# kubewharf/kubebrain

Measured on NVIDIA H100. Metric: range-scan + watch-fanout events/sec, higher is better.
Workload: dtype u8

## Files before the change

### kubebrain_b200/csrc/kb_watch.cu

```cuda
#include <algorithm>
#include <map>
#include <unordered_map>

#include "kb_internal.cuh"

struct kb_events_dev {
    DBuf keys;
    DBuf klen;
    DBuf rev;
    DBuf batch_off;
    uint32_t n = 0, nb = 0, stride = 0;
};

struct WatchTablesDev {
    uint32_t n_ids = 0, n_groups = 0, n_lens = 0, table_size = 0, max_len = 0, pstride16 = 1;
    uint64_t d_hint = 0;
    DBuf gprefix, wgroup, wminrev, lens, table;
    DBuf gstate , galloc, lists, ematch, seg, seg_sorted, bitmaps, pm, wstate ,
        wstart, total;
    DBuf arena;
    size_t tab_end = 0, scr_bytes = 0, scr_sig = 0;
    bool scratch_clean = false;
    uint32_t scratch_groups = 0, scratch_large = 0, scratch_bm_words = 0;
    uint32_t fan_gen = 0;
    uint32_t fan_set = 0;
    int fan_grid = 0;
    uint32_t wr_set = 0;
    cudaEvent_t ev_fan = nullptr, ev_write[2] = {nullptr, nullptr};
};

namespace {

constexpr unsigned FULL = 0xffffffffu;
constexpr uint64_t FNV_OFFSET = 14695981039346656037ull;
constexpr uint64_t FNV_PRIME = 1099511628211ull;

__host__ __device__ __forceinline__ uint32_t slot_of(uint64_t h, uint32_t len, uint32_t mask)
{
    uint64_t m = h ^ ((uint64_t)len * 0x9E3779B97F4A7C15ull);
    m ^= m >> 29;
    return (uint32_t)(m ^ (m >> 32)) & mask;
}

struct EvDev {
    const uint4 *keys;
    const uint32_t *klen;
    const uint64_t *rev;
    const uint64_t *batch_off;
    uint32_t n, nb, stride16;
};

struct TabDev {
    const uint4 *gprefix;
    const uint32_t *wgroup;
    const uint64_t *wminrev;
    const uint32_t *lens;
    const uint4 *table;
    uint32_t n_ids, n_groups, n_lens, mask, max_len, pstride16;
};

enum { FC_NONMONO = 0, FC_CURSOR = 1, FC_NLARGE = 2, FC_NMED = 3, FC_ARRIVE = 4, FC_GEN = 5, FC_DONE = 6, FC_ABORT = 7, FC_WORDS = 16 };
constexpr unsigned long long FAN_UNSET = ~0ull, FAN_BUSY = ~0ull - 1;
constexpr uint32_t FAN_THREADS = 384;
constexpr uint32_t BM_WORDS = 256;

struct FanScratch {
    uint32_t *gcnt, *gfill, *ctl;
    unsigned long long *galloc;
    uint32_t *med_list, *large_list;
    uint32_t *ematch, *seg, *sorted, *bitmaps;
    uint64_t *pm;
    uint32_t *wcnt, *wsrc, *wn, *wlo;
    uint64_t *wstart, *total;
    uint32_t big_t, max_large, bm_words, chunks_per_group, gen_base;
    uint32_t *z_gcnt, *z_bitmaps, *nlarge_w, *nlarge_r;
    unsigned long long *z_galloc;
    uint64_t *o_start, *h_start;
    uint64_t *h_pub, epoch;
};

__device__ __forceinline__ uint32_t ldcg32(const uint32_t *p) { return __ldcg(p); }
__device__ __forceinline__ uint64_t ldcg64(const uint64_t *p) { return __ldcg((const unsigned long long *)p); }

__device__ __forceinline__ void fan_grid_sync(uint32_t *ctl, uint32_t target)
{
    __syncthreads();
    if (threadIdx.x == 0) {
        __threadfence();
        if (atomicAdd(&ctl[FC_ARRIVE], 1u) == gridDim.x - 1) {
            atomicExch(&ctl[FC_ARRIVE], 0u);
            __threadfence();
            atomicExch(&ctl[FC_GEN], target);
        } else {
            const long long t0 = clock64();
            while (*(volatile uint32_t *)&ctl[FC_GEN] != target) {
                __nanosleep(64);
                if (clock64() - t0 > 4000000000ll) {
                    atomicExch(&ctl[FC_ABORT], 1u);
                    break;
                }
                if (*(volatile uint32_t *)&ctl[FC_ABORT]) break;
            }
        }
        __threadfence();
    }
    __syncthreads();
}

__device__ __forceinline__ void d_batch_pm(const EvDev &ev, uint64_t *__restrict__ pm, uint32_t *__restrict__ nonmono,
                                           uint32_t vblock)
{
    const uint32_t w = (vblock * blockDim.x + threadIdx.x) >> 5, lane = threadIdx.x & 31;
    if (w >= ev.nb) return;
    const uint64_t lo = ev.batch_off[w], hi = ev.batch_off[w + 1];
    uint64_t carry = 0;
    bool bad = false;
    for (uint64_t c = lo; c < hi; c += 32) {
        const uint64_t i = c + lane;
        uint64_t v = i < hi ? ev.rev[i] : 0;
        if (i < hi && i > 0 && ev.rev[i - 1] > v) bad = true;
#pragma unroll
        for (int d = 1; d < 32; d <<= 1) {
            uint64_t o = __shfl_up_sync(FULL, v, d);
            if (lane >= (unsigned)d) v = max(v, o);
        }
        v = max(v, carry);
        if (i < hi) pm[i] = v;
        carry = __shfl_sync(FULL, v, 31);
    }
    if (__any_sync(FULL, bad) && lane == 0) atomicOr(nonmono, 1u);
}

constexpr int FAN_EPT = 3;

__device__ __forceinline__ void d_match_count(const EvDev &ev, const TabDev &tb, uint32_t *__restrict__ ematch,
                                              uint32_t *__restrict__ gcnt, uint32_t vblock)
{
    const uint32_t lane = threadIdx.x & 31;
    uint32_t i[FAN_EPT], klen[FAN_EPT];
    const uint4 *kp[FAN_EPT];
    uint64_t h[FAN_EPT];
    uint4 chunk[FAN_EPT];
    bool valid[FAN_EPT];
#pragma unroll
    for (int e = 0; e < FAN_EPT; e++) {
        i[e] = (vblock * FAN_EPT + e) * blockDim.x + threadIdx.x;
        valid[e] = i[e] < ev.n;
        klen[e] = valid[e] ? ev.klen[i[e]] : 0;
        kp[e] = ev.keys + (uint64_t)(valid[e] ? i[e] : 0) * ev.stride16;
        h[e] = FNV_OFFSET;
        chunk[e] = make_uint4(0, 0, 0, 0);
    }
    uint32_t pos = 0;
    for (uint32_t li = 0; li < tb.n_lens; li++) {
        const uint32_t L = __ldg(tb.lens + li);
        for (; pos < L; pos++) {
            if ((pos & 15) == 0) {
#pragma unroll
                for (int e = 0; e < FAN_EPT; e++) chunk[e] = __ldg(kp[e] + (pos >> 4));
            }
#pragma unroll
            for (int e = 0; e < FAN_EPT; e++) h[e] = (h[e] ^ (uint64_t)byte_of(chunk[e], pos & 15)) * FNV_PRIME;
        }
        uint32_t s[FAN_EPT], g[FAN_EPT];
        uint4 t[FAN_EPT];
#pragma unroll
        for (int e = 0; e < FAN_EPT; e++) {
            s[e] = slot_of(h[e], L, tb.mask);
            t[e] = __ldg(tb.table + s[e]);
            g[e] = KB_NONE;
        }
#pragma unroll
        for (int e = 0; e < FAN_EPT; e++) {
            if (!(valid[e] && L <= klen[e])) continue;
            for (;;) {
                if (t[e].w == KB_NONE) break;
                if (t[e].x == (uint32_t)h[e] && t[e].y == (uint32_t)(h[e] >> 32) && t[e].z == L) {
                    const uint4 *gp = tb.gprefix + (uint64_t)t[e].w * tb.pstride16;
                    bool eq = true;
                    for (uint32_t k = 0; k * 16 < L && eq; k++) {
                        uint4 a = __ldg(kp[e] + k), b = __ldg(gp + k);
                        int p = first_diff16(a, b);
                        if (p < 16 && k * 16 + p < L) eq = false;
                    }
                    if (eq) {
                        g[e] = t[e].w;
                        break;
                    }
                }
                s[e] = (s[e] + 1) & tb.mask;
                t[e] = __ldg(tb.table + s[e]);
            }
        }
#pragma unroll
        for (int e = 0; e < FAN_EPT; e++) {
            if (valid[e]) ematch[(uint64_t)li * ev.n + i[e]] = g[e];
            const unsigned peers = __match_any_sync(FULL, g[e]);
            if (g[e] != KB_NONE && lane == (unsigned)(__ffs(peers) - 1)) atomicAdd(&gcnt[g[e]], (uint32_t)__popc(peers));
        }
    }
}

__device__ __forceinline__ unsigned long long d_group_alloc(const FanScratch &sc, uint32_t g)
{
    unsigned long long a = __ldcg(&sc.galloc[g]);
    if (a < FAN_BUSY) return a;
    const unsigned long long old = atomicCAS(&sc.galloc[g], FAN_UNSET, FAN_BUSY);
    if (old == FAN_UNSET) {
        const uint32_t n = ldcg32(&sc.gcnt[g]);
        uint32_t cls = KB_NONE;
        if (n > sc.big_t) {
            const uint32_t slot = atomicAdd(&sc.ctl[FC_NLARGE], 1u);
            if (slot < sc.max_large) {
                cls = slot;
                sc.large_list[slot] = g;
            }
        } else if (n > 32) {
            sc.med_list[atomicAdd(&sc.ctl[FC_NMED], 1u)] = g;
        }
        const uint32_t base = atomicAdd(&sc.ctl[FC_CURSOR], n);
        a = ((unsigned long long)cls << 32) | base;
        __threadfence();
        atomicExch(&sc.galloc[g], a);
        return a;
    }
    if (old < FAN_BUSY) return old;
    do {
        __nanosleep(32);
        a = *(volatile unsigned long long *)&sc.galloc[g];
    } while (a >= FAN_BUSY);
    return a;
}

__device__ __forceinline__ void d_scatter(const FanScratch &sc, uint32_t n_events, uint32_t n_lens, uint32_t vblock)
{
    const uint32_t i = vblock * blockDim.x + threadIdx.x;
    const uint32_t lane = threadIdx.x & 31;
    const bool valid = i < n_events;
    for (uint32_t li = 0; li < n_lens; li++) {
        const uint32_t g = valid ? ldcg32(&sc.ematch[(uint64_t)li * n_events + i]) : KB_NONE;
        const unsigned peers = __match_any_sync(FULL, g);
        if (g == KB_NONE) continue;
        const uint32_t leader = __ffs(peers) - 1;
        unsigned long long a = 0;
        uint32_t fill = 0;
        if (lane == leader) {
            a = d_group_alloc(sc, g);
            if ((uint32_t)(a >> 32) == KB_NONE) fill = atomicAdd(&sc.gfill[g], (uint32_t)__popc(peers));
        }
        const uint32_t base = __shfl_sync(peers, (uint32_t)a, leader);
        const uint32_t cls = __shfl_sync(peers, (uint32_t)(a >> 32), leader);
        fill = __shfl_sync(peers, fill, leader);
        if (cls != KB_NONE) {
            if (lane == leader) sc.bitmaps[(uint64_t)cls * sc.bm_words + (i >> 5)] = peers;
        } else {
            sc.seg[base + fill + __popc(peers & ((1u << lane) - 1))] = i;
        }
    }
}

__device__ __forceinline__ uint32_t block_excl_scan_u32(uint32_t v, uint32_t *wsum , uint32_t &total)
{
    const uint32_t lane = threadIdx.x & 31, wid = threadIdx.x >> 5, nw = blockDim.x >> 5;
    uint32_t inc = v;
#pragma unroll
    for (int d = 1; d < 32; d <<= 1) {
        uint32_t o = __shfl_up_sync(FULL, inc, d);
        if (lane >= (unsigned)d) inc += o;
    }
    if (lane == 31) wsum[wid] = inc;
    __syncthreads();
    if (threadIdx.x == 0) {
        uint32_t run = 0;
        for (uint32_t k = 0; k < nw; k++) {
            uint32_t x = wsum[k];
            wsum[k] = run;
            run += x;
        }
        wsum[32] = run;
    }
    __syncthreads();
    const uint32_t ex = wsum[wid] + inc - v;
    total = wsum[32];
    __syncthreads();
    return ex;
}

__device__ __forceinline__ void d_sort_medium(const FanScratch &sc, uint32_t *bm, uint32_t *wsum, uint32_t *red)
{
    const uint32_t nmed = ldcg32(&sc.ctl[FC_NMED]);
    for (uint32_t bi = blockIdx.x; bi < nmed; bi += gridDim.x) {
        const uint32_t g = ldcg32(&sc.med_list[bi]);
        const uint32_t n = ldcg32(&sc.gcnt[g]), base = (uint32_t)__ldcg(&sc.galloc[g]);
        if (threadIdx.x == 0) {
            red[0] = 0xFFFFFFFFu;
            red[1] = 0;
        }
        __syncthreads();
        uint32_t mn = 0xFFFFFFFFu, mx = 0;
        for (uint32_t j = threadIdx.x; j < n; j += blockDim.x) {
            const uint32_t v = ldcg32(&sc.seg[base + j]);
            mn = min(mn, v);
            mx = max(mx, v);
        }
        atomicMin(&red[0], mn);
        atomicMax(&red[1], mx);
        __syncthreads();
        mn = red[0];
        mx = red[1];
        uint32_t outpos = 0;
        for (uint64_t w0 = mn & ~31u; w0 <= mx; w0 += (uint64_t)BM_WORDS * 32) {
            const uint64_t need_words = ((uint64_t)mx - w0) / 32 + 1;
            const uint32_t nwords = need_words < BM_WORDS ? (uint32_t)need_words : BM_WORDS;
            for (uint32_t j = threadIdx.x; j < nwords; j += blockDim.x) bm[j] = 0;
            __syncthreads();
            for (uint32_t j = threadIdx.x; j < n; j += blockDim.x) {
                const uint64_t v = ldcg32(&sc.seg[base + j]);
                if (v >= w0 && v < w0 + (uint64_t)nwords * 32) {
                    const uint32_t d = (uint32_t)(v - w0);
                    atomicOr(&bm[d >> 5], 1u << (d & 31));
                }
            }
            __syncthreads();
            const uint32_t per = (nwords + blockDim.x - 1) / blockDim.x;
            const uint32_t wlo = min(nwords, threadIdx.x * per), whi = min(nwords, wlo + per);
            uint32_t cnt = 0;
            for (uint32_t j = wlo; j < whi; j++) cnt += __popc(bm[j]);
            uint32_t total;
            uint32_t at = outpos + block_excl_scan_u32(cnt, wsum, total);
            for (uint32_t j = wlo; j < whi; j++) {
                uint32_t bits = bm[j];
                while (bits) {
                    const uint32_t b = __ffs(bits) - 1;
                    bits &= bits - 1;
                    sc.sorted[base + at++] = (uint32_t)(w0 + (uint64_t)j * 32 + b);
                }
            }
            outpos += total;
            __syncthreads();
        }
        __syncthreads();
    }
}

__device__ __forceinline__ void d_expand_large(const FanScratch &sc, uint32_t *wsum, uint32_t *pre_sp)
{
    uint32_t &pre_s = *pre_sp;
    const uint32_t nlarge = min(ldcg32(&sc.ctl[FC_NLARGE]), sc.max_large);
    for (uint32_t job = blockIdx.x; job < nlarge * sc.chunks_per_group; job += gridDim.x) {
        const uint32_t slot = job / sc.chunks_per_group, chunk = job % sc.chunks_per_group;
        const uint32_t g = ldcg32(&sc.large_list[slot]);
        const uint32_t *bm = sc.bitmaps + (uint64_t)slot * sc.bm_words;
        uint32_t part = 0;
        for (uint32_t j = threadIdx.x; j < chunk * FAN_THREADS; j += blockDim.x) part += __popc(ldcg32(&bm[j]));
        uint32_t tot;
        block_excl_scan_u32(part, wsum, tot);
        if (threadIdx.x == 0) pre_s = tot;
        __syncthreads();
        const uint32_t wi = chunk * FAN_THREADS + threadIdx.x;
        uint32_t bits = wi < sc.bm_words ? ldcg32(&bm[wi]) : 0;
        uint32_t total;
        uint32_t at = (uint32_t)__ldcg(&sc.galloc[g]) + pre_s + block_excl_scan_u32(__popc(bits), wsum, total);
        while (bits) {
            const uint32_t b = __ffs(bits) - 1;
            bits &= bits - 1;
            sc.sorted[at++] = wi * 32 + b;
        }
        __syncthreads();
    }
}

__device__ __forceinline__ void d_watcher_big(const TabDev &tb, const FanScratch &sc, bool mono, uint32_t w, uint32_t n,
                                              uint32_t base, uint32_t lane)
{
    const uint64_t mr = __ldg(tb.wminrev + w);
    uint32_t lo = 0, cnt = 0;
    if (n <= 32) {
        const uint32_t v = lane < n ? ldcg32(&sc.seg[base + lane]) : 0xFFFFFFFFu;
        uint32_t rank = 0;
#pragma unroll
        for (int j = 0; j < 32; j++) {
            const uint32_t o = __shfl_sync(FULL, v, j);
            rank += (o < v) ? 1u : 0u;
        }
        if (lane < n) sc.sorted[base + rank] = v;
        const bool keep = lane < n && ldcg64(&sc.pm[v]) >= mr;
        cnt = __popc(__ballot_sync(FULL, keep));
        lo = mono ? n - cnt : 0;
    } else if (mono) {
        const uint32_t *M = sc.sorted + base;
        uint32_t hi = n;
        for (;;) {
            const uint32_t span = hi - lo;
            if (span == 0) break;
            if (span <= 32) {
                const bool ge = lane < span && ldcg64(&sc.pm[ldcg32(&M[lo + lane])]) >= mr;
                const unsigned m = __ballot_sync(FULL, ge);
                lo += m ? (uint32_t)(__ffs(m) - 1) : span;
                break;
            }
            const uint32_t piv = lo + (uint32_t)(((uint64_t)span * (lane + 1)) / 33);
            const bool ge = ldcg64(&sc.pm[ldcg32(&M[piv])]) >= mr;
            const int k = __popc(~__ballot_sync(FULL, ge));
            uint32_t nlo = lo, nhi = hi;
            if (k > 0) nlo = __shfl_sync(FULL, piv, k - 1) + 1;
            if (k < 32) nhi = __shfl_sync(FULL, piv, k);
            lo = nlo;
            hi = nhi;
        }
        cnt = n - lo;
    } else {
        const uint32_t *M = sc.sorted + base;
        for (uint32_t c = 0; c < n; c += 32) {
            const uint32_t j = c + lane;
            const bool keep = j < n && ldcg64(&sc.pm[ldcg32(&M[j])]) >= mr;
            cnt += __popc(__ballot_sync(FULL, keep));
        }
    }
    if (lane == 0) {
        sc.wcnt[w] = cnt;
        sc.wsrc[w] = base;
        sc.wn[w] = n;
        sc.wlo[w] = lo;
    }
}

__device__ __forceinline__ void d_watcher_count(const TabDev &tb, const FanScratch &sc, bool mono)
{
    const uint32_t lane = threadIdx.x & 31, half = lane >> 4, sub = lane & 15;
    const uint32_t warps = (gridDim.x * blockDim.x) >> 5;
    for (uint32_t w0 = ((blockIdx.x * blockDim.x + threadIdx.x) >> 5) * 2; w0 < tb.n_ids; w0 += warps * 2) {
        const uint32_t w = w0 + half;
        const bool have = w < tb.n_ids;
        const uint32_t g = have ? __ldg(tb.wgroup + w) : KB_NONE;
        uint32_t n = 0, base = 0;
        unsigned long long a = FAN_UNSET;
        if (g != KB_NONE) a = __ldcg(&sc.galloc[g]);
        if (a < FAN_BUSY) {
            n = ldcg32(&sc.gcnt[g]);
            base = (uint32_t)a;
        }
        const unsigned hmask = half ? 0xFFFF0000u : 0x0000FFFFu;
        if (n <= 16) {
            const uint64_t mr = have ? __ldg(tb.wminrev + w) : 0;
            const uint32_t v = sub < n ? ldcg32(&sc.seg[base + sub]) : 0xFFFFFFFFu;
            uint32_t rank = 0;
#pragma unroll
            for (int j = 0; j < 16; j++) {
                const uint32_t o = __shfl_sync(hmask, v, j, 16);
                rank += (o < v) ? 1u : 0u;
            }
            if (sub < n) sc.sorted[base + rank] = v;
            const bool keep = sub < n && ldcg64(&sc.pm[v]) >= mr;
            const uint32_t cnt = __popc(__ballot_sync(hmask, keep));
            if (sub == 0 && have) {
                sc.wcnt[w] = cnt;
                sc.wsrc[w] = base;
                sc.wn[w] = n;
                sc.wlo[w] = mono ? n - cnt : 0;
            }
        }
        __syncwarp();
        const uint32_t n0 = __shfl_sync(FULL, n, 0), n1 = __shfl_sync(FULL, n, 16);
        const uint32_t b0 = __shfl_sync(FULL, base, 0), b1 = __shfl_sync(FULL, base, 16);
        if (n0 > 16) d_watcher_big(tb, sc, mono, w0, n0, b0, lane);
        if (n1 > 16 && w0 + 1 < tb.n_ids) d_watcher_big(tb, sc, mono, w0 + 1, n1, b1, lane);
    }
}

__device__ __forceinline__ void d_finish(const TabDev &tb, const FanScratch &sc, uint64_t *ws )
{
    const uint32_t W = tb.n_ids, lane = threadIdx.x & 31, wid = threadIdx.x >> 5, nw = blockDim.x >> 5;
    const uint32_t per = ((W + nw - 1) / nw + 31) & ~31u;
    const uint32_t a = min(W, wid * per), b = min(W, a + per);
    uint64_t sum = 0;
    for (uint32_t w = a + lane; w < b; w += 32) sum += ldcg32(&sc.wcnt[w]);
#pragma unroll
    for (int d = 16; d > 0; d >>= 1) sum += __shfl_xor_sync(FULL, sum, d);
    if (lane == 0) ws[wid] = sum;
    __syncthreads();
    if (threadIdx.x == 0) {
        uint64_t run = 0;
        for (uint32_t k = 0; k < nw; k++) {
            uint64_t x = ws[k];
            ws[k] = run;
            run += x;
        }
        ws[32] = run;
    }
    __syncthreads();
    uint64_t carry = ws[wid];
    for (uint32_t w0 = a; w0 < b; w0 += 32) {
        const uint32_t w = w0 + lane;
        const uint64_t c = w < b ? ldcg32(&sc.wcnt[w]) : 0;
        uint64_t inc = c;
#pragma unroll
        for (int d = 1; d < 32; d <<= 1) {
            uint64_t o = __shfl_up_sync(FULL, inc, d);
            if (lane >= (unsigned)d) inc += o;
        }
        if (w < b) {
            const uint64_t at = carry + inc - c;
            sc.wstart[w] = at;
            sc.o_start[w] = at;
            sc.h_start[w] = at;
        }
        carry += __shfl_sync(FULL, inc, 31);
    }
    const uint32_t aborted = ldcg32(&sc.ctl[FC_ABORT]);
    if (threadIdx.x == 0) {
        sc.wstart[W] = ws[32];
        sc.o_start[W] = ws[32];
        sc.h_start[W] = ws[32];
        sc.total[0] = ws[32];
        sc.total[1] = (uint64_t)ldcg32(&sc.ctl[FC_NONMONO]) | ((uint64_t)aborted << 32);
        *sc.nlarge_w = min(ldcg32(&sc.ctl[FC_NLARGE]), sc.max_large);
    }
    __syncthreads();
    if (threadIdx.x < FC_WORDS && threadIdx.x != FC_GEN) sc.ctl[threadIdx.x] = 0;
    __threadfence_system();
    __syncthreads();
    if (threadIdx.x == 0) {
        sc.h_pub[1] = aborted;
        sc.h_pub[2] = ws[32];
        pub_raise(sc.h_pub, sc.epoch);
    }
}

__device__ __forceinline__ uint64_t fan_now_ns();

__device__ __forceinline__ uint64_t fan_now_ns()
{
    uint64_t t;
    asm volatile("mov.u64 %0, %%globaltimer;" : "=l"(t));
    return t;
}

__global__ void __maxnreg__(64)
k_fanout(EvDev ev, TabDev tb, FanScratch sc)
{
    const bool stamp = blockIdx.x == 0 && threadIdx.x == 0;
    uint64_t t_begin = 0;
    if (threadIdx.x == 0) {
        t_begin = fan_now_ns();
        atomicMax((unsigned long long *)&sc.ctl[8], (unsigned long long)t_begin);
    }
    uint64_t t_p[4] = {0, 0, 0, 0};
    __shared__ uint32_t bm[BM_WORDS];
    __shared__ uint32_t wsum[33];
    __shared__ uint32_t red[2];
    __shared__ uint64_t ws64[33];
    __shared__ uint32_t last_s;
    const uint32_t pm_blocks = (ev.nb * 32 + FAN_THREADS - 1) / FAN_THREADS;
    const uint32_t ev_blocks = tb.n_groups ? (ev.n + FAN_THREADS - 1) / FAN_THREADS : 0;
    const uint32_t ev_blocks3 = (ev_blocks + FAN_EPT - 1) / FAN_EPT;
    {
        const uint64_t tid = (uint64_t)blockIdx.x * blockDim.x + threadIdx.x, nth = (uint64_t)gridDim.x * blockDim.x;
        const uint32_t G = tb.n_groups;
        for (uint64_t i = tid; i < 2ull * (G + 1); i += nth) sc.z_gcnt[i] = 0;
        for (uint64_t i = tid; i < G; i += nth) sc.z_galloc[i] = FAN_UNSET;
        const uint64_t zb = (uint64_t)min(ldcg32(sc.nlarge_r), sc.max_large) * sc.bm_words;
        for (uint64_t i = tid; i < zb; i += nth) sc.z_bitmaps[i] = 0;
    }
    for (uint32_t vb = blockIdx.x; vb < pm_blocks + ev_blocks3; vb += gridDim.x) {
        if (vb < pm_blocks)
            d_batch_pm(ev, sc.pm, &sc.ctl[FC_NONMONO], vb);
        else
            d_match_count(ev, tb, sc.ematch, sc.gcnt, vb - pm_blocks);
    }
    fan_grid_sync(sc.ctl, sc.gen_base + 1);
    if (stamp) t_p[0] = fan_now_ns();
    for (uint32_t vb = blockIdx.x; vb < ev_blocks; vb += gridDim.x) d_scatter(sc, ev.n, tb.n_lens, vb);
    fan_grid_sync(sc.ctl, sc.gen_base + 2);
    if (stamp) t_p[1] = fan_now_ns();
    d_sort_medium(sc, bm, wsum, red);
    d_expand_large(sc, wsum, red);
    fan_grid_sync(sc.ctl, sc.gen_base + 3);
    if (stamp) t_p[2] = fan_now_ns();
    const bool mono = ldcg32(&sc.ctl[FC_NONMONO]) == 0;
    d_watcher_count(tb, sc, mono);
    if (stamp) {
        t_p[3] = fan_now_ns();
        sc.h_pub[3] = t_p[0] - t_begin;
        sc.h_pub[4] = t_p[1] - t_p[0];
        sc.h_pub[5] = t_p[2] - t_p[1];
        sc.h_pub[6] = t_p[3] - t_p[2];
        sc.h_pub[7] = __ldcg((const unsigned long long *)&sc.ctl[8]) - t_begin;
    }
    __syncthreads();
    if (threadIdx.x == 0) {
        __threadfence();
        last_s = atomicAdd(&sc.ctl[FC_DONE], 1u) == gridDim.x - 1;
        __threadfence();
    }
    __syncthreads();
    if (last_s) d_finish(tb, sc, ws64);
}

__device__ __forceinline__ void d_expand_write(uint32_t n_ids, const uint32_t *__restrict__ wsrc,
                                               const uint32_t *__restrict__ wlo, const uint32_t *__restrict__ sorted,
                                               const uint64_t *__restrict__ wstart, uint64_t n_deliveries,
                                               uint32_t *__restrict__ out)
{
    for (uint64_t d = (uint64_t)blockIdx.x * blockDim.x + threadIdx.x; d < n_deliveries;
         d += (uint64_t)gridDim.x * blockDim.x) {
        uint32_t lo = 0, hi = n_ids;
        while (hi - lo > 1) {
            const uint32_t mid = (lo + hi) >> 1;
            if (wstart[mid] <= d) lo = mid; else hi = mid;
        }
        const uint32_t w = lo;
        out[d] = sorted[wsrc[w] + wlo[w] + (uint32_t)(d - wstart[w])];
    }
}

__device__ __forceinline__ void d_expand_write_general(uint32_t n_ids, const uint64_t *__restrict__ wminrev,
                                                       const uint32_t *__restrict__ wsrc, const uint32_t *__restrict__ wn,
                                                       const uint32_t *__restrict__ sorted,
                                                       const uint64_t *__restrict__ pm,
                                                       const uint64_t *__restrict__ wstart, uint32_t *__restrict__ out)
{
    const uint32_t lane = threadIdx.x & 31;
    const uint32_t warps = (gridDim.x * blockDim.x) >> 5;
    for (uint32_t w = (blockIdx.x * blockDim.x + threadIdx.x) >> 5; w < n_ids; w += warps) {
        const uint32_t n = wn[w];
        const uint32_t *M = sorted + wsrc[w];
        const uint64_t mr = wminrev[w];
        const uint64_t o = wstart[w];
        uint64_t total = 0;
        for (uint32_t c = 0; c < n; c += 32) {
            const uint32_t j = c + lane;
            const uint32_t e = j < n ? M[j] : 0;
            const bool keep = j < n && pm[e] >= mr;
            const unsigned m = __ballot_sync(FULL, keep);
            if (keep) out[o + total + __popc(m & ((1u << lane) - 1))] = e;
            total += __popc(m);
        }
    }
}

__global__ void __launch_bounds__(256)
k_expand_write(uint32_t n_ids, const uint64_t *__restrict__ wminrev, const uint32_t *__restrict__ wsrc,
               const uint32_t *__restrict__ wn, const uint32_t *__restrict__ wlo, const uint32_t *__restrict__ sorted,
               const uint64_t *__restrict__ pm, const uint64_t *__restrict__ total ,
               const uint64_t *__restrict__ wstart, uint64_t capacity, uint32_t *__restrict__ out)
{
    const uint64_t n_deliveries = wstart[n_ids];
    if (n_deliveries > capacity) return;
    if ((total[1] >> 32) != 0) return;
    if ((uint32_t)total[1] == 0)
        d_expand_write(n_ids, wsrc, wlo, sorted, wstart, n_deliveries, out);
    else
        d_expand_write_general(n_ids, wminrev, wsrc, wn, sorted, pm, wstart, out);
}

uint64_t fnv1a(const std::string &s)
{
    uint64_t h = FNV_OFFSET;
    for (unsigned char c : s) h = (h ^ c) * FNV_PRIME;
    return h;
}

inline size_t arena_align(size_t x) { return (x + 255) & ~(size_t)255; }

void arena_view(WatchTablesDev &T, size_t &cursor, DBuf &view, size_t bytes)
{
    view.p = (uint8_t *)T.arena.p + cursor;
    view.cap = 0;
    cursor += arena_align(std::max<size_t>(bytes, 16));
}

int arena_reserve(kb_ctx *ctx, WatchTablesDev &T, size_t need)
{
    if (T.arena.p && T.arena.cap >= need) return KB_OK;
    KB_TRY(dbuf_ensure(ctx, T.arena, need + need / 2));
    T.scratch_clean = false;
    ctx->watch_dirty = true;
    cudaStreamAttrValue attr;
    memset(&attr, 0, sizeof(attr));
// ... 179 lines not shown
    w.prefix.assign((const char *)prefix, (size_t)prefix_len);
    w.min_rev = min_rev;
    w.live = true;
    if (!ctx->free_watch_ids.empty()) {
        *id = ctx->free_watch_ids.back();
        ctx->free_watch_ids.pop_back();
        ctx->watchers[*id] = w;
    } else {
        ctx->watchers.push_back(w);
        *id = (uint32_t)ctx->watchers.size() - 1;
    }
    ctx->watch_dirty = true;
    return KB_OK;
}

extern "C" int kb_watch_del(kb_ctx *ctx, uint32_t id)
{
    if (!ctx) return KB_EINVAL;
    std::lock_guard<std::mutex> g(ctx->mu);
    if (id >= ctx->watchers.size() || !ctx->watchers[id].live) return kb_fail(ctx, KB_EINVAL, "unknown watcher %u", id);
    ctx->watchers[id].live = false;
    ctx->free_watch_ids.push_back(id);
    ctx->watch_dirty = true;
    return KB_OK;
}

extern "C" int kb_watch_count(kb_ctx *ctx, uint64_t *n)
{
    if (!ctx || !n) return KB_EINVAL;
    std::lock_guard<std::mutex> g(ctx->mu);
    uint64_t c = 0;
    for (auto &w : ctx->watchers) c += w.live ? 1 : 0;
    *n = c;
    return KB_OK;
}

extern "C" int kb_events_upload(kb_ctx *ctx, const kb_events *ev, kb_events_dev **out)
{
    if (!ctx || !ev || !out || (ev->n && (!ev->keys || !ev->key_off || !ev->rev))) return KB_EINVAL;
    std::lock_guard<std::mutex> g(ctx->mu);
    cudaSetDevice(ctx->device);
    KB_TRY(lane_take(ctx));
    kb_events_dev *d = new kb_events_dev();
    int rc = events_upload_locked(ctx, ev, d);
    if (rc == KB_OK && cudaStreamSynchronize(ctx->lane().stream) != cudaSuccess) rc = kb_fail(ctx, KB_ECUDA, "event upload");
    if (rc != KB_OK) {
        events_release(d);
        delete d;
        return rc;
    }
    *out = d;
    return KB_OK;
}

extern "C" void kb_events_free(kb_ctx *ctx, kb_events_dev *ev)
{
    if (!ev) return;
    if (ctx) {
        std::lock_guard<std::mutex> g(ctx->mu);
        cudaSetDevice(ctx->device);
        cudaStreamSynchronize(ctx->lane().stream);
        events_release(ev);
    }
    delete ev;
}

__global__ void k_publish_total(const uint64_t *__restrict__ total, uint64_t *host, uint64_t epoch)
{
    if (threadIdx.x == 0) {
        host[1] = total[1] >> 32;
        host[2] = total[0];
        pub_raise(host, epoch);
    }
}

static int match_locked(kb_ctx *ctx, const kb_events_dev *d, int out_mode, kb_result **out)
{
    kb_tp tseg = kb_now();
    if (ctx->watch_dirty || !ctx->wt) {
        KB_CUDA(ctx, cudaStreamSynchronize(ctx->stream2));
        KB_TRY(rebuild_tables(ctx));
    }
    WatchTablesDev &T = *ctx->wt;
    if (d->stride < needed_stride(ctx))
        return kb_fail(ctx, KB_ESTATE, "event slab was uploaded for shorter watcher prefixes (stride %u < %u); upload again",
                       d->stride, needed_stride(ctx));
    const uint32_t E = d->n, G = T.n_groups, W = T.n_ids, NL = std::max(T.n_lens, 1u);
    const uint64_t seg_cap = std::max<uint64_t>((uint64_t)E * NL, 1);
    if (seg_cap >= 0xFFFFFFF0ull) return kb_fail(ctx, KB_ELIMIT, "events x distinct prefix lengths exceeds 2^32");
    const uint32_t big_t = std::max<uint32_t>(1024, E / 64);
    const uint32_t max_large = (uint32_t)(seg_cap / big_t) + 1;
    const uint32_t bm_words = (E + 31) / 32;
    const uint32_t chunks_per_group = (bm_words + FAN_THREADS - 1) / FAN_THREADS;
    const size_t gstate_words = (size_t)4 * (G + 1) + FC_WORDS + 4;
    const size_t bitmap_bytes = std::max<size_t>((size_t)max_large * bm_words * 4, 16);
    const size_t one[5] = {arena_align(seg_cap * 4), arena_align(std::max<size_t>((size_t)E * 8, 16)), arena_align((size_t)(W + 1) * 16),
                           arena_align((size_t)(W + 2) * 8), arena_align(16)};
    const size_t sizes[11] = {gstate_words * 4, (size_t)2 * (G + 1) * 8, 2 * bitmap_bytes, (size_t)(G + max_large + 2) * 4, seg_cap * 4,
                              seg_cap * 4, 2 * one[0], 2 * one[1], 2 * one[2], 2 * one[3], 2 * one[4]};
    size_t scr = 0, sig = 1469598103934665603ull;
    for (size_t x : sizes) {
        scr += arena_align(std::max<size_t>(x, 16));
        sig = (sig ^ x) * 1099511628211ull;
    }
    if (T.tab_end + scr > T.arena.cap) {
        KB_CUDA(ctx, cudaStreamSynchronize(ctx->stream2));
        T.scr_bytes = scr;
        KB_TRY(arena_reserve(ctx, T, T.tab_end + scr + 4096));
        KB_TRY(rebuild_tables(ctx));
    }
    T.scr_bytes = std::max(T.scr_bytes, scr);
    if (sig != T.scr_sig) T.scratch_clean = false;
    T.scr_sig = sig;
    {
        size_t cur = T.tab_end;
        DBuf *views[11] = {&T.gstate, &T.galloc, &T.bitmaps, &T.lists, &T.ematch, &T.seg, &T.seg_sorted, &T.pm, &T.wstate,
                           &T.wstart, &T.total};
        for (int i = 0; i < 11; i++) arena_view(T, cur, *views[i], sizes[i]);
    }

    EvDev ev;
    ev.keys = (const uint4 *)d->keys.p;
    ev.klen = (const uint32_t *)d->klen.p;
    ev.rev = (const uint64_t *)d->rev.p;
    ev.batch_off = (const uint64_t *)d->batch_off.p;
    ev.n = E;
    ev.nb = d->nb;
    ev.stride16 = d->stride / 16;
    TabDev tb;
    tb.gprefix = (const uint4 *)T.gprefix.p;
    tb.wgroup = (const uint32_t *)T.wgroup.p;
    tb.wminrev = (const uint64_t *)T.wminrev.p;
    tb.lens = (const uint32_t *)T.lens.p;
    tb.table = (const uint4 *)T.table.p;
    tb.n_ids = W;
    tb.n_groups = G;
    tb.n_lens = T.n_lens;
    tb.mask = T.table_size - 1;
    tb.max_len = T.max_len;
    tb.pstride16 = T.pstride16;
    FanScratch sc;
    const uint32_t set = T.fan_set & 1;
    uint32_t *gs = (uint32_t *)T.gstate.p;
    sc.gcnt = gs + (size_t)set * 2 * (G + 1);
    sc.gfill = sc.gcnt + (G + 1);
    sc.z_gcnt = gs + (size_t)(set ^ 1) * 2 * (G + 1);
    sc.ctl = gs + (size_t)4 * (G + 1);
    sc.nlarge_w = sc.ctl + FC_WORDS + set;
    sc.nlarge_r = sc.ctl + FC_WORDS + (set ^ 1);
    sc.galloc = (unsigned long long *)T.galloc.p + (size_t)set * (G + 1);
    sc.z_galloc = (unsigned long long *)T.galloc.p + (size_t)(set ^ 1) * (G + 1);
    sc.med_list = (uint32_t *)T.lists.p;
    sc.large_list = sc.med_list + G + 1;
    sc.ematch = (uint32_t *)T.ematch.p;
    sc.seg = (uint32_t *)T.seg.p;
    const uint32_t ws = T.wr_set & 1;
    sc.sorted = (uint32_t *)((uint8_t *)T.seg_sorted.p + ws * one[0]);
    sc.bitmaps = (uint32_t *)T.bitmaps.p + (size_t)set * (bitmap_bytes / 4);
    sc.z_bitmaps = (uint32_t *)T.bitmaps.p + (size_t)(set ^ 1) * (bitmap_bytes / 4);
    sc.pm = (uint64_t *)((uint8_t *)T.pm.p + ws * one[1]);
    sc.wcnt = (uint32_t *)((uint8_t *)T.wstate.p + ws * one[2]);
    sc.wsrc = sc.wcnt + (W + 1);
    sc.wn = sc.wsrc + (W + 1);
    sc.wlo = sc.wn + (W + 1);
    sc.wstart = (uint64_t *)((uint8_t *)T.wstart.p + ws * one[3]);
    sc.total = (uint64_t *)((uint8_t *)T.total.p + ws * one[4]);
    sc.big_t = big_t;
    sc.max_large = max_large;
    sc.bm_words = bm_words;
    sc.chunks_per_group = chunks_per_group;

    if (!T.scratch_clean || T.scratch_groups != G || T.scratch_large != max_large || T.scratch_bm_words != bm_words) {
        KB_CUDA(ctx, cudaMemsetAsync(T.gstate.p, 0, gstate_words * 4, ctx->lane().stream));
        KB_CUDA(ctx, cudaMemsetAsync(T.galloc.p, 0xFF, (size_t)2 * (G + 1) * 8, ctx->lane().stream));
        KB_CUDA(ctx, cudaMemsetAsync(T.bitmaps.p, 0, 2 * bitmap_bytes, ctx->lane().stream));
        T.fan_gen = 0;
        T.scratch_groups = G;
        T.scratch_large = max_large;
        T.scratch_bm_words = bm_words;
    }
    T.scratch_clean = false;
    const uint64_t ev_bytes = (uint64_t)E * (d->stride + 4);
    KB_TRY(hostpub_ensure(ctx, ctx->wpub, 64, ctx->lane().stream));
    uint64_t *h_pub = (uint64_t *)ctx->wpub.p;
    uint64_t cap = std::max<uint64_t>(T.d_hint + T.d_hint / 4 + 4096, 1 << 16);
    uint64_t D = 0;
    DBuf d_out;
    HBuf h_out;
    int rc = KB_OK;
    KB_TRY(pool_get_dev(ctx, (size_t)(W + 1) * 8 + cap * 4 + 16, &d_out));
    rc = pool_get_host(ctx, (size_t)(W + 1) * 8 + 16, &h_out);
    if (rc != KB_OK) {
        pool_put_dev(ctx, d_out);
        return rc;
    }
    if (!T.ev_fan) {
        cudaEventCreateWithFlags(&T.ev_fan, cudaEventDisableTiming);
        cudaEventCreateWithFlags(&T.ev_write[0], cudaEventDisableTiming);
        cudaEventCreateWithFlags(&T.ev_write[1], cudaEventDisableTiming);
    }
    cudaStream_t sw = ctx->stream2;
    KB_CUDA(ctx, cudaStreamWaitEvent(ctx->lane().stream, T.ev_write[ws], 0));
    const uint64_t wepoch = ++ctx->wpub.epoch;
    sc.o_start = (uint64_t *)d_out.p;
    sc.h_start = (uint64_t *)h_out.p;
    sc.h_pub = h_pub;
    sc.epoch = wepoch;
    const bool run = E && W;
    if (run) {
        if (!T.fan_grid) {
            int per_sm = 0;
            cudaOccupancyMaxActiveBlocksPerMultiprocessor(&per_sm, k_fanout, (int)FAN_THREADS, 0);
            if (per_sm < 1) {
                pool_put_dev(ctx, d_out);
                pool_put_host(ctx, h_out);
                return kb_fail(ctx, KB_ECUDA, "k_fanout does not fit on an SM");
            }
            T.fan_grid = ctx->n_sms;
        }
        sc.gen_base = T.fan_gen;
        KB_LAUNCH(ctx, "k_fanout", ev_bytes + (uint64_t)E * NL * 12 + (uint64_t)E * 16 + (uint64_t)W * 44,
                  (k_fanout<<<(unsigned)T.fan_grid, FAN_THREADS, 0, ctx->lane().stream>>>(ev, tb, sc)));
        T.fan_gen += 3;
        T.fan_set ^= 1;
    } else {
        cudaMemsetAsync(sc.wstart, 0, (size_t)(W + 2) * 8, ctx->lane().stream);
        cudaMemsetAsync(sc.total, 0, 16, ctx->lane().stream);
        cudaMemsetAsync(d_out.p, 0, (size_t)(W + 1) * 8, ctx->lane().stream);
        memset(h_out.p, 0, (size_t)(W + 1) * 8);
        k_publish_total<<<1, 32, 0, ctx->lane().stream>>>(sc.total, h_pub, wepoch);
    }
    auto launch_write = [&](uint32_t *o_idx, uint64_t capacity) {
        const uint64_t cap_grid = (uint64_t)ctx->n_sms * 16;
        const unsigned wgrid = (unsigned)std::max<uint64_t>(std::min<uint64_t>((capacity + 255) / 256, cap_grid),
                                                            std::min<uint64_t>(((uint64_t)W * 32 + 255) / 256, cap_grid));
        KB_LAUNCH_S(ctx, sw, "k_expand_write", capacity * 8,
                    (k_expand_write<<<wgrid, 256, 0, sw>>>(W, tb.wminrev, sc.wsrc, sc.wn, sc.wlo, sc.sorted, sc.pm, sc.total,
                                                          sc.wstart, capacity, o_idx)));
    };
    cudaEventRecord(T.ev_fan, ctx->lane().stream);
    cudaStreamWaitEvent(sw, T.ev_fan, 0);
    if (run) launch_write((uint32_t *)((uint64_t *)d_out.p + W + 1), cap);
    T.wr_set ^= 1;
    kb_seg(ctx, "host:match_launch", tseg);
    rc = hostpub_wait(ctx, ctx->wpub, wepoch, ctx->lane().stream, "watch match");
    kb_seg(ctx, "host:match_sync", tseg);
    if (rc == KB_OK && ctx->wpub.err()) rc = kb_fail(ctx, KB_ECUDA, "watch match: a grid barrier timed out");
    if (rc != KB_OK) {
        pool_put_dev(ctx, d_out);
        pool_put_host(ctx, h_out);
        return rc;
    }
    D = h_pub[2];
    T.d_hint = D;
    if (ctx->prof_on && run) {
        static const char *names[5] = {"fan:P1_match", "fan:P2_scatter", "fan:P3_sort", "fan:P4_watchers", "fan:last_cta_start"};
        for (int i = 0; i < 5; i++) {
// ... 94 lines not shown
```

Before: 2.497 billion.

## Replace lazy group allocation and final watcher scan with grid-barrier scan and decoupled look-back

Per-group offsets are no longer allocated lazily through CAS spin-waits during scatter. The last block to arrive at the first grid barrier now computes them with a block-wide scan over group counts. Watcher counting moves to ticketed ranges of 96 watchers, whose offsets are resolved through a decoupled look-back prefix scan. This removes the single-block serial pass over all watcher counts in the finish step. In exchange, one block scans all groups serially while the rest of the grid waits at the barrier, and look-back adds spin-polling between blocks.

```diff
diff --git a/kubebrain_b200/csrc/kb_watch.cu b/kubebrain_b200/csrc/kb_watch.cu
--- a/kubebrain_b200/csrc/kb_watch.cu
+++ b/kubebrain_b200/csrc/kb_watch.cu
@@ -59,8 +59,9 @@
     uint32_t n_ids, n_groups, n_lens, mask, max_len, pstride16;
 };
 
-enum { FC_NONMONO = 0, FC_CURSOR = 1, FC_NLARGE = 2, FC_NMED = 3, FC_ARRIVE = 4, FC_GEN = 5, FC_DONE = 6, FC_ABORT = 7, FC_WORDS = 16 };
-constexpr unsigned long long FAN_UNSET = ~0ull, FAN_BUSY = ~0ull - 1;
+enum { FC_NONMONO = 0, FC_WTICKET = 1, FC_NLARGE = 2, FC_NMED = 3, FC_ARRIVE = 4, FC_GEN = 5, FC_DONE = 6, FC_ABORT = 7, FC_WORDS = 16 };
+constexpr uint32_t FAN_WRANGE = 96;
+constexpr unsigned long long LB_AGG = 1ull << 62, LB_INC = 2ull << 62, LB_VAL = LB_AGG - 1;
 constexpr uint32_t FAN_THREADS = 384;
 constexpr uint32_t BM_WORDS = 256;
 
@@ -70,11 +71,11 @@
     uint32_t *med_list, *large_list;
     uint32_t *ematch, *seg, *sorted, *bitmaps;
     uint64_t *pm;
-    uint32_t *wcnt, *wsrc, *wn, *wlo;
+    uint32_t *wsrc, *wn, *wlo;
     uint64_t *wstart, *total;
-    uint32_t big_t, max_large, bm_words, chunks_per_group, gen_base;
+    uint32_t big_t, max_large, bm_words, chunks_per_group, gen_base, n_ranges;
     uint32_t *z_gcnt, *z_bitmaps, *nlarge_w, *nlarge_r;
-    unsigned long long *z_galloc;
+    unsigned long long *look, *z_look;
     uint64_t *o_start, *h_start;
     uint64_t *h_pub, epoch;
 };
@@ -82,29 +83,41 @@
 __device__ __forceinline__ uint32_t ldcg32(const uint32_t *p) { return __ldcg(p); }
 __device__ __forceinline__ uint64_t ldcg64(const uint64_t *p) { return __ldcg((const unsigned long long *)p); }
 
-__device__ __forceinline__ void fan_grid_sync(uint32_t *ctl, uint32_t target)
+template <class Last>
+__device__ __forceinline__ bool fan_grid_sync(uint32_t *ctl, uint32_t target, uint32_t *bar_s , Last last)
 {
     __syncthreads();
     if (threadIdx.x == 0) {
         __threadfence();
-        if (atomicAdd(&ctl[FC_ARRIVE], 1u) == gridDim.x - 1) {
+        bar_s[0] = atomicAdd(&ctl[FC_ARRIVE], 1u) == gridDim.x - 1;
+    }
+    __syncthreads();
+    if (bar_s[0]) {
+        last();
+        __threadfence();
+        __syncthreads();
+        if (threadIdx.x == 0) {
             atomicExch(&ctl[FC_ARRIVE], 0u);
             __threadfence();
             atomicExch(&ctl[FC_GEN], target);
-        } else {
-            const long long t0 = clock64();
-            while (*(volatile uint32_t *)&ctl[FC_GEN] != target) {
-                __nanosleep(64);
-                if (clock64() - t0 > 4000000000ll) {
-                    atomicExch(&ctl[FC_ABORT], 1u);
-                    break;
-                }
-                if (*(volatile uint32_t *)&ctl[FC_ABORT]) break;
+        }
+    } else if (threadIdx.x == 0) {
+        const long long t0 = clock64();
+        while (*(volatile uint32_t *)&ctl[FC_GEN] != target) {
+            __nanosleep(64);
+            if (clock64() - t0 > 4000000000ll) {
+                atomicExch(&ctl[FC_ABORT], 1u);
+                break;
             }
-        }
+            if (*(volatile uint32_t *)&ctl[FC_ABORT]) break;
+        }
+    }
+    if (threadIdx.x == 0) {
         __threadfence();
+        bar_s[1] = *(volatile uint32_t *)&ctl[FC_ABORT];
     }
     __syncthreads();
+    return bar_s[1] != 0;
 }
 
 __device__ __forceinline__ void d_batch_pm(const EvDev &ev, uint64_t *__restrict__ pm, uint32_t *__restrict__ nonmono,
@@ -201,37 +214,6 @@
     }
 }
 
-__device__ __forceinline__ unsigned long long d_group_alloc(const FanScratch &sc, uint32_t g)
-{
-    unsigned long long a = __ldcg(&sc.galloc[g]);
-    if (a < FAN_BUSY) return a;
-    const unsigned long long old = atomicCAS(&sc.galloc[g], FAN_UNSET, FAN_BUSY);
-    if (old == FAN_UNSET) {
-        const uint32_t n = ldcg32(&sc.gcnt[g]);
-        uint32_t cls = KB_NONE;
-        if (n > sc.big_t) {
-            const uint32_t slot = atomicAdd(&sc.ctl[FC_NLARGE], 1u);
-            if (slot < sc.max_large) {
-                cls = slot;
-                sc.large_list[slot] = g;
-            }
-        } else if (n > 32) {
-            sc.med_list[atomicAdd(&sc.ctl[FC_NMED], 1u)] = g;
-        }
-        const uint32_t base = atomicAdd(&sc.ctl[FC_CURSOR], n);
-        a = ((unsigned long long)cls << 32) | base;
-        __threadfence();
-        atomicExch(&sc.galloc[g], a);
-        return a;
-    }
-    if (old < FAN_BUSY) return old;
-    do {
-        __nanosleep(32);
-        a = *(volatile unsigned long long *)&sc.galloc[g];
-    } while (a >= FAN_BUSY);
-    return a;
-}
-
 __device__ __forceinline__ void d_scatter(const FanScratch &sc, uint32_t n_events, uint32_t n_lens, uint32_t vblock)
 {
     const uint32_t i = vblock * blockDim.x + threadIdx.x;
@@ -245,7 +227,7 @@
         unsigned long long a = 0;
         uint32_t fill = 0;
         if (lane == leader) {
-            a = d_group_alloc(sc, g);
+            a = __ldcg(&sc.galloc[g]);
             if ((uint32_t)(a >> 32) == KB_NONE) fill = atomicAdd(&sc.gfill[g], (uint32_t)__popc(peers));
         }
         const uint32_t base = __shfl_sync(peers, (uint32_t)a, leader);
@@ -284,6 +266,54 @@
     total = wsum[32];
     __syncthreads();
     return ex;
+}
+
+constexpr uint32_t FAN_SCAN_V = 4;
+
+__device__ __forceinline__ void d_group_scan(const FanScratch &sc, uint32_t G, uint32_t *wsum )
+{
+    const uint4 *c4 = (const uint4 *)sc.gcnt;
+    const uint32_t per = (G + 4 * blockDim.x - 1) / (4 * blockDim.x) * 4;
+    const uint32_t a = min(G, threadIdx.x * per), b = min(G, a + per);
+    uint32_t sum = 0;
+    for (uint32_t g0 = a; g0 < b; g0 += 4 * FAN_SCAN_V) {
+        uint4 v[FAN_SCAN_V];
+#pragma unroll
+        for (uint32_t j = 0; j < FAN_SCAN_V; j++) v[j] = g0 + 4 * j < b ? __ldcg(c4 + g0 / 4 + j) : make_uint4(0, 0, 0, 0);
+#pragma unroll
+        for (uint32_t j = 0; j < FAN_SCAN_V; j++) {
+            const uint32_t g = g0 + 4 * j;
+            sum += (g < b ? v[j].x : 0) + (g + 1 < b ? v[j].y : 0) + (g + 2 < b ? v[j].z : 0) + (g + 3 < b ? v[j].w : 0);
+        }
+    }
+    uint32_t total;
+    uint32_t at = block_excl_scan_u32(sum, wsum, total);
+    for (uint32_t g0 = a; g0 < b; g0 += 4 * FAN_SCAN_V) {
+        uint4 v[FAN_SCAN_V];
+#pragma unroll
+        for (uint32_t j = 0; j < FAN_SCAN_V; j++) v[j] = g0 + 4 * j < b ? __ldcg(c4 + g0 / 4 + j) : make_uint4(0, 0, 0, 0);
+#pragma unroll
+        for (uint32_t j = 0; j < FAN_SCAN_V; j++) {
+            const uint32_t n4[4] = {v[j].x, v[j].y, v[j].z, v[j].w};
+#pragma unroll
+            for (uint32_t k = 0; k < 4; k++) {
+                const uint32_t g = g0 + 4 * j + k, n = n4[k];
+                if (g >= b) continue;
+                uint32_t cls = KB_NONE;
+                if (n > sc.big_t) {
+                    const uint32_t slot = atomicAdd(&sc.ctl[FC_NLARGE], 1u);
+                    if (slot < sc.max_large) {
+                        cls = slot;
+                        sc.large_list[slot] = g;
+                    }
+                } else if (n > 32) {
+                    sc.med_list[atomicAdd(&sc.ctl[FC_NMED], 1u)] = g;
+                }
+                sc.galloc[g] = ((unsigned long long)cls << 32) | at;
+                at += n;
+            }
+        }
+    }
 }
 
 __device__ __forceinline__ void d_sort_medium(const FanScratch &sc, uint32_t *bm, uint32_t *wsum, uint32_t *red)
@@ -371,7 +401,7 @@
 }
 
 __device__ __forceinline__ void d_watcher_big(const TabDev &tb, const FanScratch &sc, bool mono, uint32_t w, uint32_t n,
-                                              uint32_t base, uint32_t lane)
+                                              uint32_t base, uint32_t lane, uint32_t *cnt_s)
 {
     const uint64_t mr = __ldg(tb.wminrev + w);
     uint32_t lo = 0, cnt = 0;
@@ -418,27 +448,26 @@
         }
     }
     if (lane == 0) {
-        sc.wcnt[w] = cnt;
+        *cnt_s = cnt;
         sc.wsrc[w] = base;
         sc.wn[w] = n;
         sc.wlo[w] = lo;
     }
 }
 
-__device__ __forceinline__ void d_watcher_count(const TabDev &tb, const FanScratch &sc, bool mono)
+__device__ __forceinline__ void d_watcher_count(const TabDev &tb, const FanScratch &sc, bool mono, uint32_t r0, uint32_t r1,
+                                                uint32_t *cnt_s)
 {
     const uint32_t lane = threadIdx.x & 31, half = lane >> 4, sub = lane & 15;
-    const uint32_t warps = (gridDim.x * blockDim.x) >> 5;
-    for (uint32_t w0 = ((blockIdx.x * blockDim.x + threadIdx.x) >> 5) * 2; w0 < tb.n_ids; w0 += warps * 2) {
+    const uint32_t warps = blockDim.x >> 5;
+    for (uint32_t w0 = r0 + (threadIdx.x >> 5) * 2; w0 < r1; w0 += warps * 2) {
         const uint32_t w = w0 + half;
-        const bool have = w < tb.n_ids;
+        const bool have = w < r1;
         const uint32_t g = have ? __ldg(tb.wgroup + w) : KB_NONE;
         uint32_t n = 0, base = 0;
-        unsigned long long a = FAN_UNSET;
-        if (g != KB_NONE) a = __ldcg(&sc.galloc[g]);
-        if (a < FAN_BUSY) {
+        if (g != KB_NONE) {
             n = ldcg32(&sc.gcnt[g]);
-            base = (uint32_t)a;
+            base = (uint32_t)__ldcg(&sc.galloc[g]);
         }
         const unsigned hmask = half ? 0xFFFF0000u : 0x0000FFFFu;
         if (n <= 16) {
@@ -454,7 +483,7 @@
             const bool keep = sub < n && ldcg64(&sc.pm[v]) >= mr;
             const uint32_t cnt = __popc(__ballot_sync(hmask, keep));
             if (sub == 0 && have) {
-                sc.wcnt[w] = cnt;
+                cnt_s[w - r0] = cnt;
                 sc.wsrc[w] = base;
                 sc.wn[w] = n;
                 sc.wlo[w] = mono ? n - cnt : 0;
@@ -463,56 +492,81 @@
         __syncwarp();
         const uint32_t n0 = __shfl_sync(FULL, n, 0), n1 = __shfl_sync(FULL, n, 16);
         const uint32_t b0 = __shfl_sync(FULL, base, 0), b1 = __shfl_sync(FULL, base, 16);
-        if (n0 > 16) d_watcher_big(tb, sc, mono, w0, n0, b0, lane);
-        if (n1 > 16 && w0 + 1 < tb.n_ids) d_watcher_big(tb, sc, mono, w0 + 1, n1, b1, lane);
-    }
-}
-
-__device__ __forceinline__ void d_finish(const TabDev &tb, const FanScratch &sc, uint64_t *ws )
-{
-    const uint32_t W = tb.n_ids, lane = threadIdx.x & 31, wid = threadIdx.x >> 5, nw = blockDim.x >> 5;
-    const uint32_t per = ((W + nw - 1) / nw + 31) & ~31u;
-    const uint32_t a = min(W, wid * per), b = min(W, a + per);
-    uint64_t sum = 0;
-    for (uint32_t w = a + lane; w < b; w += 32) sum += ldcg32(&sc.wcnt[w]);
-#pragma unroll
-    for (int d = 16; d > 0; d >>= 1) sum += __shfl_xor_sync(FULL, sum, d);
-    if (lane == 0) ws[wid] = sum;
+        if (n0 > 16) d_watcher_big(tb, sc, mono, w0, n0, b0, lane, &cnt_s[w0 - r0]);
+        if (n1 > 16 && w0 + 1 < r1) d_watcher_big(tb, sc, mono, w0 + 1, n1, b1, lane, &cnt_s[w0 + 1 - r0]);
+    }
+}
+
+__device__ __forceinline__ uint64_t d_look_back(unsigned long long *look, uint32_t r, uint64_t agg)
+{
+    const uint32_t lane = threadIdx.x & 31;
+    volatile unsigned long long *vl = look;
+    if (lane == 0) vl[r] = (r == 0 ? LB_INC : LB_AGG) | agg;
+    uint64_t prev = 0;
+    for (int64_t j = (int64_t)r - 1; j >= 0; j -= 32) {
+        const int64_t k = j - lane;
+        unsigned long long v;
+        for (;;) {
+            v = k >= 0 ? vl[k] : (unsigned long long)LB_INC;
+            if (__all_sync(FULL, v >= LB_AGG)) break;
+            __nanosleep(32);
+        }
+        const unsigned inc = __ballot_sync(FULL, v >= LB_INC);
+        const uint32_t stop = inc ? __ffs(inc) - 1 : 31;
+        uint64_t x = lane <= stop ? (v & LB_VAL) : 0;
+#pragma unroll
+        for (int d = 16; d > 0; d >>= 1) x += __shfl_xor_sync(FULL, x, d);
+        prev += x;
+        if (inc) break;
+    }
+    if (lane == 0 && r > 0) vl[r] = LB_INC | (prev + agg);
+    return prev;
+}
+
+__device__ __forceinline__ void d_range_offsets(const FanScratch &sc, uint32_t r, uint32_t r0, uint32_t r1,
+                                                const uint32_t *cnt_s, uint64_t *ws )
+{
+    const uint32_t lane = threadIdx.x & 31, wid = threadIdx.x >> 5, nw = blockDim.x >> 5;
+    const bool mine = threadIdx.x < r1 - r0;
+    const uint64_t c = mine ? cnt_s[threadIdx.x] : 0;
+    uint64_t inc = c;
+#pragma unroll
+    for (int d = 1; d < 32; d <<= 1) {
+        const uint64_t o = __shfl_up_sync(FULL, inc, d);
+        if (lane >= (unsigned)d) inc += o;
+    }
+    if (lane == 31) ws[wid] = inc;
     __syncthreads();
-    if (threadIdx.x == 0) {
-        uint64_t run = 0;
-        for (uint32_t k = 0; k < nw; k++) {
-            uint64_t x = ws[k];
-            ws[k] = run;
-            run += x;
-        }
-        ws[32] = run;
+    if (wid == 0) {
+        const uint64_t x = lane < nw ? ws[lane] : 0;
+        uint64_t xi = x;
+#pragma unroll
+        for (int d = 1; d < 32; d <<= 1) {
+            const uint64_t o = __shfl_up_sync(FULL, xi, d);
+            if (lane >= (unsigned)d) xi += o;
+        }
+        const uint64_t prev = d_look_back(sc.look, r, __shfl_sync(FULL, xi, 31));
+        if (lane < nw) ws[lane] = prev + xi - x;
     }
     __syncthreads();
-    uint64_t carry = ws[wid];
-    for (uint32_t w0 = a; w0 < b; w0 += 32) {
-        const uint32_t w = w0 + lane;
-        const uint64_t c = w < b ? ldcg32(&sc.wcnt[w]) : 0;
-        uint64_t inc = c;
-#pragma unroll
-        for (int d = 1; d < 32; d <<= 1) {
-            uint64_t o = __shfl_up_sync(FULL, inc, d);
-            if (lane >= (unsigned)d) inc += o;
-        }
-        if (w < b) {
-            const uint64_t at = carry + inc - c;
-            sc.wstart[w] = at;
-            sc.o_start[w] = at;
-            sc.h_start[w] = at;
-        }
-        carry += __shfl_sync(FULL, inc, 31);
-    }
+    if (mine) {
+        const uint64_t at = ws[wid] + inc - c;
+        sc.wstart[r0 + threadIdx.x] = at;
+        sc.o_start[r0 + threadIdx.x] = at;
+        sc.h_start[r0 + threadIdx.x] = at;
+    }
+}
+
+__device__ __forceinline__ void d_finish(const TabDev &tb, const FanScratch &sc)
+{
+    const uint32_t W = tb.n_ids;
+    const uint64_t D = __ldcg(&sc.look[sc.n_ranges - 1]) & LB_VAL;
     const uint32_t aborted = ldcg32(&sc.ctl[FC_ABORT]);
     if (threadIdx.x == 0) {
-        sc.wstart[W] = ws[32];
-        sc.o_start[W] = ws[32];
-        sc.h_start[W] = ws[32];
-        sc.total[0] = ws[32];
+        sc.wstart[W] = D;
+        sc.o_start[W] = D;
+        sc.h_start[W] = D;
+        sc.total[0] = D;
         sc.total[1] = (uint64_t)ldcg32(&sc.ctl[FC_NONMONO]) | ((uint64_t)aborted << 32);
         *sc.nlarge_w = min(ldcg32(&sc.ctl[FC_NLARGE]), sc.max_large);
     }
@@ -522,7 +576,7 @@
     __syncthreads();
     if (threadIdx.x == 0) {
         sc.h_pub[1] = aborted;
-        sc.h_pub[2] = ws[32];
+        sc.h_pub[2] = D;
         pub_raise(sc.h_pub, sc.epoch);
     }
 }
@@ -550,7 +604,7 @@
     __shared__ uint32_t wsum[33];
     __shared__ uint32_t red[2];
     __shared__ uint64_t ws64[33];
-    __shared__ uint32_t last_s;
+    __shared__ uint32_t last_s, ticket_s, bar_s[2];
     const uint32_t pm_blocks = (ev.nb * 32 + FAN_THREADS - 1) / FAN_THREADS;
     const uint32_t ev_blocks = tb.n_groups ? (ev.n + FAN_THREADS - 1) / FAN_THREADS : 0;
     const uint32_t ev_blocks3 = (ev_blocks + FAN_EPT - 1) / FAN_EPT;
@@ -558,7 +612,7 @@
         const uint64_t tid = (uint64_t)blockIdx.x * blockDim.x + threadIdx.x, nth = (uint64_t)gridDim.x * blockDim.x;
         const uint32_t G = tb.n_groups;
         for (uint64_t i = tid; i < 2ull * (G + 1); i += nth) sc.z_gcnt[i] = 0;
-        for (uint64_t i = tid; i < G; i += nth) sc.z_galloc[i] = FAN_UNSET;
+        for (uint64_t i = tid; i < sc.n_ranges; i += nth) sc.z_look[i] = 0;
         const uint64_t zb = (uint64_t)min(ldcg32(sc.nlarge_r), sc.max_large) * sc.bm_words;
         for (uint64_t i = tid; i < zb; i += nth) sc.z_bitmaps[i] = 0;
     }
@@ -568,17 +622,32 @@
         else
             d_match_count(ev, tb, sc.ematch, sc.gcnt, vb - pm_blocks);
     }
-    fan_grid_sync(sc.ctl, sc.gen_base + 1);
+    bool aborted = fan_grid_sync(sc.ctl, sc.gen_base + 1, bar_s, [&] { d_group_scan(sc, tb.n_groups, wsum); });
     if (stamp) t_p[0] = fan_now_ns();
-    for (uint32_t vb = blockIdx.x; vb < ev_blocks; vb += gridDim.x) d_scatter(sc, ev.n, tb.n_lens, vb);
-    fan_grid_sync(sc.ctl, sc.gen_base + 2);
+    if (!aborted)
+        for (uint32_t vb = blockIdx.x; vb < ev_blocks; vb += gridDim.x) d_scatter(sc, ev.n, tb.n_lens, vb);
+    aborted |= fan_grid_sync(sc.ctl, sc.gen_base + 2, bar_s, [] {});
     if (stamp) t_p[1] = fan_now_ns();
-    d_sort_medium(sc, bm, wsum, red);
-    d_expand_large(sc, wsum, red);
-    fan_grid_sync(sc.ctl, sc.gen_base + 3);
+    if (!aborted) {
+        d_sort_medium(sc, bm, wsum, red);
+        d_expand_large(sc, wsum, red);
+    }
+    aborted |= fan_grid_sync(sc.ctl, sc.gen_base + 3, bar_s, [] {});
     if (stamp) t_p[2] = fan_now_ns();
     const bool mono = ldcg32(&sc.ctl[FC_NONMONO]) == 0;
-    d_watcher_count(tb, sc, mono);
+    bool wrote = false;
+    while (!aborted) {
+        __syncthreads();
+        if (threadIdx.x == 0) ticket_s = atomicAdd(&sc.ctl[FC_WTICKET], 1u);
+        __syncthreads();
+        const uint32_t r = ticket_s;
+        if (r >= sc.n_ranges) break;
+        const uint32_t r0 = r * FAN_WRANGE, r1 = min(tb.n_ids, r0 + FAN_WRANGE);
+        d_watcher_count(tb, sc, mono, r0, r1, bm);
+        __syncthreads();
+        d_range_offsets(sc, r, r0, r1, bm, ws64);
+        wrote = threadIdx.x < FAN_WRANGE;
+    }
     if (stamp) {
         t_p[3] = fan_now_ns();
         sc.h_pub[3] = t_p[0] - t_begin;
@@ -587,6 +656,7 @@
         sc.h_pub[6] = t_p[3] - t_p[2];
         sc.h_pub[7] = __ldcg((const unsigned long long *)&sc.ctl[8]) - t_begin;
     }
+    if (wrote || stamp) __threadfence_system();
     __syncthreads();
     if (threadIdx.x == 0) {
         __threadfence();
@@ -594,7 +664,7 @@
         __threadfence();
     }
     __syncthreads();
-    if (last_s) d_finish(tb, sc, ws64);
+    if (last_s) d_finish(tb, sc);
 }
 
 __device__ __forceinline__ void d_expand_write(uint32_t n_ids, const uint32_t *__restrict__ wsrc,
@@ -940,9 +1010,10 @@
         KB_TRY(rebuild_tables(ctx));
     }
     WatchTablesDev &T = *ctx->wt;
-    if (d->stride < needed_stride(ctx))
+    const uint32_t need_stride = std::max<uint32_t>(16, (T.max_len + 15) / 16 * 16);
+    if (d->stride < need_stride)
         return kb_fail(ctx, KB_ESTATE, "event slab was uploaded for shorter watcher prefixes (stride %u < %u); upload again",
-                       d->stride, needed_stride(ctx));
+                       d->stride, need_stride);
     const uint32_t E = d->n, G = T.n_groups, W = T.n_ids, NL = std::max(T.n_lens, 1u);
     const uint64_t seg_cap = std::max<uint64_t>((uint64_t)E * NL, 1);
     if (seg_cap >= 0xFFFFFFF0ull) return kb_fail(ctx, KB_ELIMIT, "events x distinct prefix lengths exceeds 2^32");
@@ -950,11 +1021,14 @@
     const uint32_t max_large = (uint32_t)(seg_cap / big_t) + 1;
     const uint32_t bm_words = (E + 31) / 32;
     const uint32_t chunks_per_group = (bm_words + FAN_THREADS - 1) / FAN_THREADS;
-    const size_t gstate_words = (size_t)4 * (G + 1) + FC_WORDS + 4;
+    const uint32_t n_ranges = (W + FAN_WRANGE - 1) / FAN_WRANGE;
+    const size_t set_words = ((size_t)2 * (G + 1) + 3) & ~(size_t)3;
+    const size_t look_word = 2 * set_words + FC_WORDS + 4;
+    const size_t gstate_words = look_word + (size_t)4 * n_ranges;
     const size_t bitmap_bytes = std::max<size_t>((size_t)max_large * bm_words * 4, 16);
-    const size_t one[5] = {arena_align(seg_cap * 4), arena_align(std::max<size_t>((size_t)E * 8, 16)), arena_align((size_t)(W + 1) * 16),
+    const size_t one[5] = {arena_align(seg_cap * 4), arena_align(std::max<size_t>((size_t)E * 8, 16)), arena_align((size_t)(W + 1) * 12),
                            arena_align((size_t)(W + 2) * 8), arena_align(16)};
-    const size_t sizes[11] = {gstate_words * 4, (size_t)2 * (G + 1) * 8, 2 * bitmap_bytes, (size_t)(G + max_large + 2) * 4, seg_cap * 4,
+    const size_t sizes[11] = {gstate_words * 4, (size_t)(G + 1) * 8, 2 * bitmap_bytes, (size_t)(G + max_large + 2) * 4, seg_cap * 4,
                               seg_cap * 4, 2 * one[0], 2 * one[1], 2 * one[2], 2 * one[3], 2 * one[4]};
     size_t scr = 0, sig = 1469598103934665603ull;
     for (size_t x : sizes) {
@@ -1000,14 +1074,16 @@
     FanScratch sc;
     const uint32_t set = T.fan_set & 1;
     uint32_t *gs = (uint32_t *)T.gstate.p;
-    sc.gcnt = gs + (size_t)set * 2 * (G + 1);
+    sc.gcnt = gs + (size_t)set * set_words;
     sc.gfill = sc.gcnt + (G + 1);
-    sc.z_gcnt = gs + (size_t)(set ^ 1) * 2 * (G + 1);
-    sc.ctl = gs + (size_t)4 * (G + 1);
+    sc.z_gcnt = gs + (size_t)(set ^ 1) * set_words;
+    sc.ctl = gs + 2 * set_words;
     sc.nlarge_w = sc.ctl + FC_WORDS + set;
     sc.nlarge_r = sc.ctl + FC_WORDS + (set ^ 1);
-    sc.galloc = (unsigned long long *)T.galloc.p + (size_t)set * (G + 1);
-    sc.z_galloc = (unsigned long long *)T.galloc.p + (size_t)(set ^ 1) * (G + 1);
+    sc.look = (unsigned long long *)(gs + look_word) + (size_t)set * n_ranges;
+    sc.z_look = (unsigned long long *)(gs + look_word) + (size_t)(set ^ 1) * n_ranges;
+    sc.n_ranges = n_ranges;
+    sc.galloc = (unsigned long long *)T.galloc.p;
     sc.med_list = (uint32_t *)T.lists.p;
     sc.large_list = sc.med_list + G + 1;
     sc.ematch = (uint32_t *)T.ematch.p;
@@ -1017,8 +1093,7 @@
     sc.bitmaps = (uint32_t *)T.bitmaps.p + (size_t)set * (bitmap_bytes / 4);
     sc.z_bitmaps = (uint32_t *)T.bitmaps.p + (size_t)(set ^ 1) * (bitmap_bytes / 4);
     sc.pm = (uint64_t *)((uint8_t *)T.pm.p + ws * one[1]);
-    sc.wcnt = (uint32_t *)((uint8_t *)T.wstate.p + ws * one[2]);
-    sc.wsrc = sc.wcnt + (W + 1);
+    sc.wsrc = (uint32_t *)((uint8_t *)T.wstate.p + ws * one[2]);
     sc.wn = sc.wsrc + (W + 1);
     sc.wlo = sc.wn + (W + 1);
     sc.wstart = (uint64_t *)((uint8_t *)T.wstart.p + ws * one[3]);
@@ -1030,7 +1105,6 @@
 
     if (!T.scratch_clean || T.scratch_groups != G || T.scratch_large != max_large || T.scratch_bm_words != bm_words) {
         KB_CUDA(ctx, cudaMemsetAsync(T.gstate.p, 0, gstate_words * 4, ctx->lane().stream));
-        KB_CUDA(ctx, cudaMemsetAsync(T.galloc.p, 0xFF, (size_t)2 * (G + 1) * 8, ctx->lane().stream));
         KB_CUDA(ctx, cudaMemsetAsync(T.bitmaps.p, 0, 2 * bitmap_bytes, ctx->lane().stream));
         T.fan_gen = 0;
         T.scratch_groups = G;
```

After: 2.488 billion (median of 6 runs). No clear change (-0.4%).
